# Nicolo2277/Vivim

Measured on AMD Instinct MI355X. Metric: frames/sec fwd+bwd, 256x256 clip=5 3-class, higher is better.
Workload: dtype bf16

## Files before the change

### vivim_amd/_lib.py

```python
import collections
import ctypes
import os
import re
import subprocess

import torch

_HERE = os.path.dirname(os.path.abspath(__file__))
CSRC = os.path.join(_HERE, "csrc")
SO_PATH = os.environ.get("VIVIM_LIB") or os.path.join(CSRC, "libvivim_hip.so")
HEADER = os.path.join(os.path.dirname(_HERE), "include", "vivim_hip.h")
EXT_HEADER = os.path.join(os.path.dirname(_HERE), "include", "vivim_hip_ext.h")

i32, i64, vp = ctypes.c_int32, ctypes.c_int64, ctypes.c_void_p

STRUCT_NAMES = {
    "vivim_ssm_fwd_params": "SsmFwdParams", "vivim_ssm_bwd_params": "SsmBwdParams",
    "vivim_conv_fwd_params": "ConvFwdParams", "vivim_conv_bwd_params": "ConvBwdParams",
    "vivim_dwconv_params": "DwConvParams", "vivim_dwconv_wgrad_params": "DwConvWgradParams",
    "vivim_dir_params": "DirParams", "vivim_conv_update_params": "ConvUpdateParams",
    "vivim_state_update_params": "StateUpdateParams", "vivim_layernorm_params": "LayerNormParams",
    "vivim_wgrad_nt_params": "WgradNtParams", "vivim_add_layernorm_params": "AddLayerNormParams",
    "vivim_seg_loss_params": "SegLossParams", "vivim_seg_metrics_params": "SegMetricsParams",
    "vivim_upsample_params": "UpsampleParams",
# ... 143 lines not shown
    if _lib is None:
        if not os.path.exists(SO_PATH):
            raise ImportError(
                f"{SO_PATH} is missing: run `python -c 'import __graft_entry__ as g; g.build()'` "
                "(or `make -C vivim_amd/csrc`). vivim_amd has no fallback path.")
        L = ctypes.CDLL(SO_PATH)
        for name, e in ALL_ENTRY_POINTS.items():
            fn = getattr(L, name)
            fn.argtypes = ([ctypes.POINTER(e.struct)] if e.struct else []) + list(e.extra) + ([vp] if e.stream else [])
            fn.restype = e.restype
        if L.vivim_abi_version() != ABI_VERSION:
            raise ImportError("libvivim_hip.so ABI version mismatch")
        for which, st in enumerate(STRUCTS):
            if L.vivim_sizeof(which) != ctypes.sizeof(st):
                raise ImportError(f"struct layout mismatch for {st.__name__}: "
                                  f"C {L.vivim_sizeof(which)} vs ctypes {ctypes.sizeof(st)}")
        _lib = L
    return _lib


_ISIZE = {F32: 4, F16: 2, BF16: 2}


def algorithmic_bytes(name, P):
    name = name.removesuffix("_det")
    f = P.f if isinstance(P, (SsmBwdParams, ConvBwdParams)) else P
    if name.startswith("vivim_opt"):
        if name.endswith("finalise"):
            return 8 * P.total_blocks + 4 * OPT_STATE_WORDS
        n = sum(P.numel[i] for i in range(P.count) if P.grads[i])
        if name.endswith("_mw"):
            return 2 * n + 8 * P.n_blocks if name.endswith("stats_mw") else 28 * n
        return 4 * n + 8 * P.n_blocks if name.endswith("stats") else 28 * n
    if name.startswith("vivim_add_layernorm"):
        n = P.batch * P.seqlen * P.channels
        if not P.weight:
            return n * ((2 if name.endswith("fwd") else 1) * _ISIZE[P.itype] + _ISIZE[P.btype])
        if name.endswith("fwd"):
            return n * (2 * _ISIZE[P.itype] + _ISIZE[P.btype] + _ISIZE[P.otype]) + 8 * P.batch * P.seqlen + 8 * P.channels
        res = (_ISIZE[P.itype] if P.dres else 0) + (_ISIZE[P.otype] if P.dy else 0) + (_ISIZE[P.btype] if P.dbranch else 0)
        return n * (2 * _ISIZE[P.itype] + res) + 8 * P.batch * P.seqlen + 12 * P.channels
    if name.startswith("vivim_token_add_norm"):
        n, b, r = P.rows * P.channels, _ISIZE[P.btype], _ISIZE[P.rtype]
        stats = 8 * P.rows if P.mean and P.weight else 0
        small = (4 * (P.rows // P.rows_per_sample) if P.scale else 0) + (4 * P.channels if P.weight else 0)
        if name.endswith("fwd"):
            small += 4 * P.channels if P.weight and P.bias else 0
            return n * (b + (r if P.res else 0) + (r if P.res_out else 0) + (b if P.weight else 0)) + stats + small
        norm = bool(P.weight and P.dy)
        small += (4 * P.channels if norm and P.dweight else 0) + (4 * P.channels if norm and P.dbias else 0)
        return (n * ((r + b if norm else 0) + (r if P.dres else 0) + (r if P.dres_in else 0) + (b if P.dbranch else 0))
                + (stats if norm else 0) + small)
    if name.startswith("vivim_token_layernorm"):
        n = P.rows * P.channels
        stats = 8 * P.rows if P.mean else 0
        if name.endswith("fwd"):
            return n * (_ISIZE[P.itype] + _ISIZE[P.otype]) + stats
        return n * (2 * _ISIZE[P.itype] + _ISIZE[P.otype]) + stats + 12 * P.channels
    if name.startswith("vivim_decode_head"):
        px = sum(P.map_h[s] * P.map_w[s] for s in range(P.n_maps))
        return (P.batch * (px * P.hidden + P.classes * P.out_h * P.out_w) * _ISIZE[P.itype]
                + 4 * (P.hidden + P.classes * P.hidden + P.classes))
    if name.startswith("vivim_head_concat"):
        px = P.out_h * P.out_w
        maps = sum(P.map_c[s] * (P.map_h[s] * P.map_w[s] + px) for s in range(P.n_maps)) * _ISIZE[P.itype]
        return P.batch * (maps + sum(P.map_c[s] * px for s in range(P.n_maps) if P.keep[s]))
    if name.startswith("vivim_upsample"):
        return P.batch * P.channels * (P.in_h * P.in_w + P.out_h * P.out_w) * _ISIZE[P.itype]
    if name.startswith("vivim_seg_metrics"):
        n = P.batch * P.pixels
        return n * (P.classes * _ISIZE[P.itype] + (8 if P.ttype == 0 else 1) + (1 if P.pred else 0)) + 12 * P.batch * P.classes
    if name.startswith("vivim_structure_loss"):
        n = P.batch * P.height * P.width
        return (n * ((2 if name.endswith("bwd") else 1) * P.classes * _ISIZE[P.itype] + (8 if P.ttype == 0 else 1))
                + 12 * P.batch * P.classes)
    if name.startswith("vivim_seg_loss"):
        n = P.batch * P.pixels
        return (n * ((2 if name.endswith("bwd") else 1) * P.classes * _ISIZE[P.itype] + (8 if P.ttype == 0 else 1))
                + 8 * P.batch * P.classes)
    if name.startswith("vivim_binary_metrics"):
        n = P.batch * P.height * P.width
        return (3 * n * (_ISIZE[P.ptype] + _ISIZE.get(P.gtype, 1)) + P.batch * (72 + (4096 if P.hist else 0))
                + (160 if P.state else 0))
    if name.startswith("vivim_selective_scan"):
        s = _ISIZE[f.itype]
        act = f.batch * f.dim * f.seqlen * s
        bc = (f.batch * f.n_groups * f.dstate * f.seqlen) if f.is_variable_B else f.dim * f.dstate
        has_z = bool(f.z)
        if name.endswith("fwd_lean"):
            return (4 if has_z else 3) * act + 2 * bc * (s if f.is_variable_B else 4) + 4 * (f.dim * f.dstate + 2 * f.dim)
        if name.endswith("fwd"):
            n_act = 3 + (2 if has_z else 0)
            return n_act * act + 2 * bc * (s if f.is_variable_B else 4) + 4 * (f.dim * f.dstate + 2 * f.dim)
        n_act = 5 + (3 if has_z else 0) + (1 if (has_z and f.out_z) else 0)
        return (n_act * act + 2 * bc * (s if f.is_variable_B else 4) + 2 * bc * 4
                + 4 * (2 * f.dim * f.dstate + 4 * f.dim))
    if name.endswith("_update"):
        return 0
    if name.startswith("vivim_dir"):
        return 4 * P.batch * P.channels * P.seqlen * _ISIZE[P.itype]
    if name.startswith("vivim_dwconv"):
        act = P.batch * P.depth * P.height * P.width * P.channels * _ISIZE[P.itype]
        return 2 * act + 4 * P.channels * (P.kd * 9 + 1)
    if name.startswith("vivim_layernorm"):
        n = P.batch * P.seqlen * P.channels
        if name.endswith("fwd"):
            return n * (_ISIZE[P.itype] + _ISIZE[P.otype]) + 8 * P.batch * P.seqlen + 8 * P.channels
        return n * (2 * _ISIZE[P.itype] + _ISIZE[P.otype]) + 8 * P.batch * P.seqlen + 12 * P.channels
    if name.startswith("vivim_wgrad"):
        return P.groups * ((P.m + P.n) * P.k * _ISIZE[P.itype] + 4 * P.m * P.n)
    s = _ISIZE[f.itype]
    act = f.batch * f.dim * f.seqlen * s
    if name.endswith("fwd"):
        return 2 * act + 4 * f.dim * (f.width + 1)
    return 3 * act + 8 * f.dim * (f.width + 1)


_profile = None
_event_pool = []
_PROFILED = ("vivim_selective_scan_fwd", "vivim_selective_scan_bwd", "vivim_causal_conv1d_fwd",
             "vivim_causal_conv1d_bwd")


def profile_begin(all_kernels=False):
    global _profile
    _profile = ([], bool(all_kernels))


def profile_end():
    global _profile
    rec = _profile[0] if _profile else []
    _profile = None
    out = []
    for name, nbytes, e0, e1 in rec:
        e1.synchronize()
        out.append((name, nbytes, e0.elapsed_time(e1) * 1e-3))
        _event_pool.extend((e0, e1))
    return out


def _event():
    if _event_pool:
        return _event_pool.pop()
    return torch.cuda.Event(enable_timing=True)


GUARD = os.environ.get("VIVIM_GUARD", "0") not in ("0", "")
_GUARD_BYTES = 1 << 16
_guards = []


def _guarded_storage(nbytes, device):
    buf = torch.full((nbytes + 2 * _GUARD_BYTES,), 0xA5, dtype=torch.uint8, device=device)
    _guards.append(buf)
    return buf[_GUARD_BYTES:_GUARD_BYTES + nbytes]


def empty(shape, dtype, device):
    if not GUARD:
        return torch.empty(shape, dtype=dtype, device=device)
    n = 1
    for d in shape:
        n *= d
    return _guarded_storage(n * torch.empty((), dtype=dtype).element_size(), device).view(dtype).view(shape)


# ... 71 lines not shown
```

### vivim_amd/csrc/capi.hip

```cpp
#include <hip/hip_runtime.h>
#include <float.h>
#include <stdarg.h>
#include <stddef.h>
#include <stdio.h>
#include <string.h>
#include <type_traits>
#include "ops.cuh"

using vivim::Launch;
using vivim::conv_channel_last;
using vivim::elem_bytes;
using vivim::vec_elems;

static thread_local char g_err[512] = "";

static int fail(int code, const char* fmt, ...) {
    va_list ap;
    va_start(ap, fmt);
    vsnprintf(g_err, sizeof(g_err), fmt, ap);
    va_end(ap);
    return code;
}

#define VCHECK(cond)                                                                   \
// ... 917 lines not shown
                    (long long)out_image);
    for (int s = 0; s < p->n_maps; ++s) {
        const int64_t image = (int64_t)p->map_c[s] * p->map_h[s] * p->map_w[s], mask = (int64_t)p->map_c[s] * p->out_h * p->out_w;
        const int64_t have = bwd ? p->dmap_batch_stride[s] : p->map_batch_stride[s];
        if (have < image)
            return fail(VIVIM_ERR_INVALID, "%s: %s[%d] = %lld: an image of map %d has %lld elements", fn,
                        bwd ? "dmap_batch_stride" : "map_batch_stride", s, (long long)have, s, (long long)image);
        if (p->keep[s] != nullptr && p->keep_batch_stride[s] < mask)
            return fail(VIVIM_ERR_INVALID, "%s: keep_batch_stride[%d] = %lld: a mask of map %d has %lld bytes", fn, s,
                        (long long)p->keep_batch_stride[s], s, (long long)mask);
    }
    bool fits = out_image <= INT32_MAX - 256 && (int64_t)p->batch * p->out_h <= INT32_MAX;
    for (int s = 0; s < p->n_maps; ++s)
        fits = fits && (2 * (int64_t)p->map_h[s] + 3) * p->out_h <= INT32_MAX && (2 * (int64_t)p->map_w[s] + 3) * p->out_w <= INT32_MAX;
    if (!fits || vivim::head_concat_blocks(*p, bwd) > INT32_MAX)
        return fail(VIVIM_ERR_INVALID, "%s: batch = %d, out (%d, %d), out_pixel_stride = %lld: the index range overflows int32", fn, p->batch,
                    p->out_h, p->out_w, (long long)p->out_pixel_stride);
    return VIVIM_OK;
}

int vivim_head_concat_fwd(const vivim_head_concat_params* p, void* stream) {
    const char* fn = "head_concat_fwd";
    if (int rc = check_head_concat(p, fn, false)) return rc;
    if (!vivim::head_concat_dispatch(*p, false, as_stream(stream)))
        return fail(VIVIM_ERR_UNSUPPORTED, "%s not implemented for type %d", fn, p->itype);
    return after_launch(fn);
}

int vivim_head_concat_bwd(const vivim_head_concat_params* p, void* stream) {
    const char* fn = "head_concat_bwd";
    if (int rc = check_head_concat(p, fn, true)) return rc;
    if (!vivim::head_concat_dispatch(*p, true, as_stream(stream)))
        return fail(VIVIM_ERR_UNSUPPORTED, "%s not implemented for type %d", fn, p->itype);
    return after_launch(fn);
}


static int check_binary_metrics(const vivim_binary_metrics_params* p, const char* fn) {
    if (p == nullptr) return fail(VIVIM_ERR_INVALID, "%s: params is NULL", fn);
    if (int rc = check_struct_bytes(fn, "vivim_binary_metrics_params", p->struct_bytes, sizeof(*p))) return rc;
    if (!dtype_ok(p->ptype)) return fail(VIVIM_ERR_INVALID, "%s: ptype = %d: pred is fp32 / fp16 / bf16 (0 / 1 / 2)", fn, p->ptype);
    if (!dtype_ok(p->gtype) && p->gtype != 3)
        return fail(VIVIM_ERR_INVALID, "%s: gtype = %d: gt is fp32 / fp16 / bf16 (0 / 1 / 2) or uint8 / bool (3)", fn, p->gtype);
    if (p->batch <= 0 || p->height <= 0 || p->width <= 0)
        return fail(VIVIM_ERR_INVALID, "%s: batch = %d, height = %d, width = %d: every size must be positive", fn, p->batch, p->height, p->width);
    const int64_t pixels = (int64_t)p->height * p->width;
    if (pixels < 2) return fail(VIVIM_ERR_INVALID, "%s: height * width = %lld: the metrics need at least 2 pixels", fn, (long long)pixels);
    if (pixels > INT32_MAX - 4096 || (int64_t)p->batch * 32 > INT32_MAX)
        return fail(VIVIM_ERR_INVALID, "%s: batch = %d, height * width = %lld: the index range overflows int32", fn, p->batch, (long long)pixels);
    if (p->pred_batch_stride < pixels || p->gt_batch_stride < pixels)
        return fail(VIVIM_ERR_INVALID, "%s: pred_batch_stride = %lld, gt_batch_stride = %lld: an image has %lld elements", fn,
                    (long long)p->pred_batch_stride, (long long)p->gt_batch_stride, (long long)pixels);
    return VIVIM_OK;
}

size_t vivim_binary_metrics_workspace_bytes(const vivim_binary_metrics_params* p) {
    if (check_binary_metrics(p, "binary_metrics_workspace_bytes") != VIVIM_OK) return 0;
    return vivim::binary_metrics_workspace_bytes(*p);
}

int vivim_binary_metrics(const vivim_binary_metrics_params* p, void* stream) {
    const char* fn = "binary_metrics";
    if (int rc = check_binary_metrics(p, fn)) return rc;
    if (p->pred == nullptr || !aligned(p->pred, elem_bytes(p->ptype)))
        return fail(VIVIM_ERR_INVALID, "%s: pred at %p: need a %d-byte aligned pointer", fn, p->pred, elem_bytes(p->ptype));
    const int gbytes = p->gtype == 3 ? 1 : elem_bytes(p->gtype);
    if (p->gt == nullptr || !aligned(p->gt, gbytes))
        return fail(VIVIM_ERR_INVALID, "%s: gt at %p: need a %d-byte aligned pointer", fn, p->gt, gbytes);
    if (p->thresholds == nullptr || !aligned(p->thresholds, 4))
        return fail(VIVIM_ERR_INVALID, "%s: thresholds at %p: need 256 fp32 thresholds at a 4-byte aligned pointer", fn, p->thresholds);
    if (p->values == nullptr || !aligned(p->values, 8))
        return fail(VIVIM_ERR_INVALID, "%s: values at %p: need an 8-byte aligned pointer to (batch, 9) fp64", fn, p->values);
    if (p->hist != nullptr && !aligned(p->hist, 4))
        return fail(VIVIM_ERR_INVALID, "%s: hist at %p: need NULL or a 4-byte aligned pointer", fn, p->hist);
    if (p->state != nullptr && !aligned(p->state, 8))
        return fail(VIVIM_ERR_INVALID, "%s: state at %p: need NULL or an 8-byte aligned pointer to 10 fp64", fn, p->state);
    const size_t need = vivim::binary_metrics_workspace_bytes(*p);
    if (int rc = check_workspace(fn, "vivim_binary_metrics_workspace_bytes", p->workspace, p->workspace_bytes, 8, need)) return rc;
    if (!vivim::binary_metrics_dispatch(*p, as_stream(stream)))
        return fail(VIVIM_ERR_UNSUPPORTED, "%s not implemented for type %d", fn, p->ptype);
    return after_launch(fn);
}

}
```

### vivim_amd/csrc/ops.cuh

```cuda
#pragma once
#include "det.cuh"
#include "../../include/vivim_hip_ext.h"
#include "../../include/vivim_hip_ext_head.h"
#include "../../include/vivim_hip_ext_binary_metrics.h"

namespace vivim {

inline bool conv_channel_last(const vivim_conv_fwd_params& f) { return f.x_c_stride == 1 && f.x_l_stride > 1; }
bool conv_fwd_dispatch(const vivim_conv_fwd_params&, hipStream_t);
bool conv_bwd_dispatch(const vivim_conv_bwd_params&, hipStream_t);
size_t conv_bwd_det_workspace_bytes(const vivim_conv_fwd_params&);
Launch conv_bwd_det_dispatch(const vivim_conv_bwd_params&, void* ws, size_t bytes, hipStream_t);
bool conv_cl_fwd_dispatch(const vivim_conv_fwd_params&, hipStream_t);
bool conv_cl_bwd_dispatch(const vivim_conv_bwd_params&, hipStream_t);
size_t conv_cl_bwd_det_slots(const vivim_conv_fwd_params&);
bool conv_cl_bwd_det_launch(const vivim_conv_bwd_params&, hipStream_t);

bool ssm_fwd_dispatch(const vivim_ssm_fwd_params&, hipStream_t);
bool ssm_fwd_lean_dispatch(const vivim_ssm_fwd_params&, void* last_state, hipStream_t);
bool ssm_bwd_dispatch(const vivim_ssm_bwd_params&, hipStream_t);
Launch ssm_bwd_det_dispatch(const vivim_ssm_bwd_params&, void* det_ws, size_t det_ws_bytes, hipStream_t);
int scan_chunk_len(int itype);
int scan_ckpt_len(const vivim_ssm_fwd_params&);
size_t scan_fwd_workspace_bytes(const vivim_ssm_fwd_params&);
size_t scan_bwd_workspace_bytes(const vivim_ssm_fwd_params&);
size_t scan_bwd_det_workspace_bytes(const vivim_ssm_fwd_params&);
size_t scan_bwd_det_call_workspace_bytes(const vivim_ssm_bwd_params&);

void conv_update_launch(const vivim_conv_update_params&, hipStream_t);
void state_update_launch(const vivim_state_update_params&, hipStream_t);

bool dwconv_fwd_dispatch(const vivim_dwconv_params&, hipStream_t);
bool dwconv_wgrad_dispatch(const vivim_dwconv_wgrad_params&, hipStream_t);
size_t dwconv_wgrad_det_workspace_bytes(const vivim_dwconv_wgrad_params&);
Launch dwconv_wgrad_det_dispatch(const vivim_dwconv_wgrad_params&, void* ws, size_t bytes, hipStream_t);

template <bool GATHER> bool dir_dispatch(const vivim_dir_params&, hipStream_t);

bool layernorm_dispatch(const vivim_layernorm_params&, bool bwd, hipStream_t);
size_t layernorm_bwd_workspace_bytes(const vivim_layernorm_params&);
bool add_layernorm_dispatch(const vivim_add_layernorm_params&, bool bwd, hipStream_t);
size_t add_layernorm_bwd_workspace_bytes(const vivim_add_layernorm_params&);

bool token_layernorm_dispatch(const vivim_token_layernorm_params&, bool bwd, hipStream_t);
bool token_layernorm_pair_ok(int itype, int otype);
size_t token_layernorm_bwd_workspace_bytes(const vivim_token_layernorm_params&);
bool token_add_norm_dispatch(const vivim_token_add_norm_params&, bool bwd, hipStream_t);
bool token_add_norm_pair_ok(int btype, int rtype);
size_t token_add_norm_bwd_workspace_bytes(const vivim_token_add_norm_params&);

bool wgrad_nt_dispatch(const vivim_wgrad_nt_params&, hipStream_t);

bool seg_loss_dispatch(const vivim_seg_loss_params&, bool bwd, hipStream_t);
size_t seg_loss_workspace_bytes(const vivim_seg_loss_params&);
bool seg_metrics_dispatch(const vivim_seg_metrics_params&, hipStream_t);
size_t seg_metrics_workspace_bytes(const vivim_seg_metrics_params&);
bool structure_loss_dispatch(const vivim_structure_loss_params&, bool bwd, hipStream_t);
size_t structure_loss_workspace_bytes(const vivim_structure_loss_params&);
int64_t structure_loss_tiles(const vivim_structure_loss_params&);

bool upsample_dispatch(const vivim_upsample_params&, bool bwd, hipStream_t);
int64_t upsample_blocks(const vivim_upsample_params&, bool bwd);
bool decode_head_dispatch(const vivim_decode_head_params&, hipStream_t);
int64_t decode_head_blocks(const vivim_decode_head_params&);
int decode_head_max_hidden();

bool head_concat_dispatch(const vivim_head_concat_params&, bool bwd, hipStream_t);
int64_t head_concat_blocks(const vivim_head_concat_params&, bool bwd);

bool binary_metrics_dispatch(const vivim_binary_metrics_params&, hipStream_t);
size_t binary_metrics_workspace_bytes(const vivim_binary_metrics_params&);

void opt_grad_stats_launch(const vivim_opt_step_params&, hipStream_t);
void opt_finalise_launch(const vivim_opt_step_params&, hipStream_t);
void opt_adamw_launch(const vivim_opt_step_params&, hipStream_t);
void opt_grad_stats_mw_launch(const vivim_opt_step_params&, int dtype, hipStream_t);
void opt_adamw_mw_launch(const vivim_opt_step_params&, const void* masters, int dtype, hipStream_t);

}
```

### vivim_amd/vivim.py

```python
import math

import os

import torch
import torch.nn as nn
import torch.nn.functional as F

from . import decode_head as _dh
from . import dwconv as _dw
from . import head_concat as _hc
from . import layernorm as _ln
from . import upsample as _up
from .mamba_simple import Mamba


class DropPath(nn.Module):

    def __init__(self, drop_prob=0.0):
        super().__init__()
        self.drop_prob = drop_prob

    def forward(self, x):
        if self.drop_prob == 0.0 or not self.training:
            return x
        keep = 1.0 - self.drop_prob
        mask = x.new_empty((x.shape[0],) + (1,) * (x.dim() - 1)).bernoulli_(keep).div_(keep)
        return x * mask

    def sample_scale(self, x):
        if self.drop_prob == 0.0 or not self.training:
            return None
        keep = 1.0 - self.drop_prob
        return torch.empty(x.shape[0], dtype=torch.float32, device=x.device).bernoulli_(keep).div_(keep)


def _init_weights(m):
    if isinstance(m, nn.Linear):
        nn.init.trunc_normal_(m.weight, std=0.02)
        if m.bias is not None:
            nn.init.constant_(m.bias, 0)
    elif isinstance(m, nn.LayerNorm):
        nn.init.constant_(m.bias, 0)
        nn.init.constant_(m.weight, 1.0)
    elif isinstance(m, nn.Conv2d):
        fan_out = m.kernel_size[0] * m.kernel_size[1] * m.out_channels // m.groups
        m.weight.data.normal_(0, math.sqrt(2.0 / fan_out))
        if m.bias is not None:
            m.bias.data.zero_()


class LayerNorm(nn.Module):

    def __init__(self, normalized_shape, eps=1e-6, data_format="channels_last"):
        super().__init__()
        if data_format not in ("channels_last", "channels_first"):
            raise NotImplementedError
        self.weight = nn.Parameter(torch.ones(normalized_shape))
        self.bias = nn.Parameter(torch.zeros(normalized_shape))
        self.eps = eps
        self.data_format = data_format
        self.normalized_shape = (normalized_shape,)

    def forward(self, x):
        if self.data_format == "channels_last":
            return F.layer_norm(x, self.normalized_shape, self.weight, self.bias, self.eps)
        mean = x.mean(1, keepdim=True)
        var = (x - mean).pow(2).mean(1, keepdim=True)
        x = (x - mean) / torch.sqrt(var + self.eps)
        return self.weight[:, None, None] * x + self.bias[:, None, None]


class DWConv(nn.Module):

    def __init__(self, dim=768):
        super().__init__()
        self.dwconv = nn.Conv3d(dim, dim, 3, 1, 1, bias=True, groups=dim)

    def forward(self, x, nf, H, W):
        B, _, C = x.shape
        if _dw.supported(x, self.dwconv.weight):
            return _dw.depthwise_conv_tokens(x, self.dwconv.weight, self.dwconv.bias, nf, H, W)
        x = self.dwconv(x.transpose(1, 2).view(B, C, nf, H, W))
        return x.flatten(2).transpose(1, 2)


class Mlp(nn.Module):
    def __init__(self, in_features, hidden_features=None, out_features=None, act_layer=nn.GELU, drop=0.0):
        super().__init__()
        out_features = out_features or in_features
        hidden_features = hidden_features or in_features
        self.fc1 = nn.Linear(in_features, hidden_features)
        self.dwconv = DWConv(hidden_features)
        self.act = act_layer()
        self.fc2 = nn.Linear(hidden_features, out_features)
        self.drop = nn.Dropout(drop)
        self.apply(_init_weights)

    def forward(self, x, nf, H, W):
        x = self.fc1(x)
        conv = self.dwconv.dwconv
        if isinstance(self.act, nn.GELU) and self.act.approximate == "none" and _dw.supported(x, conv.weight) \
                and not os.environ.get("VIVIM_NO_DWCONV_GELU"):
            x = self.drop(_dw.depthwise_conv_gelu_tokens(x, conv.weight, conv.bias, nf, H, W))
        else:
            x = self.drop(self.act(self.dwconv(x, nf, H, W)))
        return self.drop(self.fc2(x))


class MambaLayer(nn.Module):

    def __init__(self, dim, d_state=16, d_conv=4, expand=2, mlp_ratio=4, drop=0.0, drop_path=0.0,
                 act_layer=nn.GELU, fused_add_norm=False):
        super().__init__()
        self.dim = dim
        self.fused_add_norm = fused_add_norm
        self.norm1 = nn.LayerNorm(dim)
        self.mamba = Mamba(d_model=dim, d_state=d_state, d_conv=d_conv, expand=expand, bimamba_type="v3")
        self.drop_path = DropPath(drop_path) if drop_path > 0.0 else nn.Identity()
        self.norm2 = nn.LayerNorm(dim)
        self.mlp = Mlp(in_features=dim, hidden_features=int(dim * mlp_ratio), act_layer=act_layer, drop=drop)
        self.apply(_init_weights)

    @staticmethod
    def _norm(norm, x_flat):
        if (_ln.supported(x_flat, norm.weight) and _ln.worthwhile(x_flat)
                and not os.environ.get("VIVIM_NO_FUSED_LAYERNORM")):
            return _ln.layer_norm_cm(x_flat, norm.weight, norm.bias, norm.eps)
        return norm(x_flat)

    def forward(self, x):
        B, C, nf, H, W = x.shape
        assert C == self.dim
        x_flat = x.reshape(B, C, nf * H * W).transpose(-1, -2)
        branch = self.mamba(self._norm(self.norm1, x_flat), nframes=nf)
        if self.fused_add_norm and self._add_norm_applies(x_flat, branch, self.norm2.weight):
            x_flat, h = _ln.add_layer_norm_cm(x_flat, branch, self.norm2.weight, self.norm2.bias, self.norm2.eps,
                                              self._drop_scale(x_flat))
            branch = self.mlp(h, nf, H, W)
            if self._add_norm_applies(x_flat, branch, None):
                x_flat = _ln.add_cm(x_flat, branch, self._drop_scale(x_flat))
            else:
                x_flat = x_flat + self.drop_path(branch)
            return x_flat.transpose(-1, -2).reshape(B, C, nf, H, W)
        x_flat = x_flat + self.drop_path(branch)
        x_flat = x_flat + self.drop_path(self.mlp(self._norm(self.norm2, x_flat), nf, H, W))
        return x_flat.transpose(-1, -2).reshape(B, C, nf, H, W)

    @staticmethod
    def _add_norm_applies(x_flat, branch, weight):
        return (_ln.add_norm_supported(x_flat, branch, weight) and _ln.worthwhile(x_flat)
                and not os.environ.get("VIVIM_NO_FUSED_LAYERNORM"))

    def _drop_scale(self, x_flat):
        return self.drop_path.sample_scale(x_flat) if isinstance(self.drop_path, DropPath) else None


def _encoder_parts(backbone):
    seg = backbone.segformer
    if hasattr(seg, "encoder"):
        enc = seg.encoder
        return list(enc.patch_embeddings), list(enc.block), list(enc.layer_norm)
    return ([s.patch_embeddings for s in seg.stages], [s.blocks for s in seg.stages],
            [s.layer_norm for s in seg.stages])


class _TokenDWConv2d(nn.Module):

    def __init__(self, hf_module):
        super().__init__()
        self.dwconv = hf_module.dwconv

    def forward(self, hidden_states, height, width):
        if _dw.supported(hidden_states, self.dwconv.weight):
            return _dw.depthwise_conv_tokens(hidden_states, self.dwconv.weight, self.dwconv.bias, 1, height, width)
        b, _, c = hidden_states.shape
        y = self.dwconv(hidden_states.transpose(1, 2).view(b, c, height, width))
        return y.flatten(2).transpose(1, 2)


def _swap_backbone_dwconv(module):
    n = 0
    for m in module.modules():
        inner = getattr(m, "dwconv", None)
        conv = getattr(inner, "dwconv", None)
        if isinstance(conv, nn.Conv2d) and conv.groups == conv.in_channels and conv.kernel_size == (3, 3) \
                and conv.stride == (1, 1) and conv.padding == (1, 1) and not isinstance(inner, _TokenDWConv2d):
            m.dwconv = _TokenDWConv2d(inner)
            n += 1
    return n


def _swap_backbone_droppath(module):
    n = 0
    for m in module.modules():
        dp = getattr(m, "drop_path", None)
        if isinstance(dp, nn.Module) and type(dp).__name__ == "SegformerDropPath":
            m.drop_path = DropPath(float(dp.drop_prob))
            n += 1
    return n


class _BackboneLayerNorm(nn.LayerNorm):
    low_precision_out = False

    @classmethod
    def adopt(cls, norm, low_precision_out):
        new = cls(norm.normalized_shape, eps=norm.eps, elementwise_affine=False)
        new.elementwise_affine = norm.elementwise_affine
        new.weight, new.bias = norm.weight, norm.bias
        new.low_precision_out = low_precision_out
        new.train(norm.training)
        return new

    def forward(self, x):
        w, b = self.weight, self.bias
        if os.environ.get("VIVIM_NO_FUSED_LAYERNORM") or w is None or len(self.normalized_shape) != 1:
            return super().forward(x)
        low = torch.get_autocast_dtype("cuda") if self.low_precision_out and x.is_cuda and torch.is_autocast_enabled("cuda") else None
        if _ln.supported(x, w) and _ln.worthwhile(x):
            return _ln.layer_norm_cm(x, w, b, self.eps, out_dtype=low if low == x.dtype else None)
        rows = _ln.tm_rows(x, w, b)
        if rows is not None and _ln.tm_worthwhile(x):
            return _ln.layer_norm_tm(x, w, b, self.eps, out_dtype=low if low is not None and _ln.tm_pair_ok(x.dtype, low) else None,
                                     rows=rows)
        return super().forward(x)


def _swap_backbone_layernorm(encoder):
    n = 0
    for root, low in ((encoder.patch_embeddings, False), (encoder.block, True)):
        for m in root.modules():
            for name, child in list(m.named_children()):
                if isinstance(child, nn.LayerNorm) and not isinstance(child, _BackboneLayerNorm):
                    setattr(m, name, _BackboneLayerNorm.adopt(child, low))
                    n += 1
    return n


class _Encoder(nn.Module):

    def __init__(self, backbone):
        super().__init__()
        pe, blocks, norms = _encoder_parts(backbone)
        self.patch_embeddings = nn.ModuleList(pe)
        self.block = nn.ModuleList(blocks)
        self.layer_norm = nn.ModuleList(norms)


def _run_block(blk, hs, height, width):
    out = blk(hs, height, width)
    return out[0] if isinstance(out, (tuple, list)) else out


def _block_norms(blk):
    for first, second in (("layernorm_before", "layernorm_after"), ("layer_norm_1", "layer_norm_2")):
        n1, n2 = getattr(blk, first, None), getattr(blk, second, None)
        if isinstance(n1, nn.LayerNorm) and isinstance(n2, nn.LayerNorm):
            ok = all(isinstance(getattr(blk, name, None), nn.Module) for name in ("attention", "mlp", "drop_path"))
            return (n1, n2) if ok else None
    return None


def _add_rows(res, branch, drop_path, norm=None):
    if not isinstance(drop_path, (DropPath, nn.Identity)):
        return None
    w = b = None
    if norm is not None:
        w, b = norm.weight, norm.bias
        if w is None or len(norm.normalized_shape) != 1:
            return None
        want = torch.get_autocast_dtype("cuda") if res.is_cuda and torch.is_autocast_enabled("cuda") else res.dtype
        if branch.dtype != want:
            return None
    rows = _ln.tm_add_rows(res, branch, w, b)
    return rows if rows is not None and _ln.tm_add_worthwhile(res) else None


def _add_norm_site(res, branch, drop_path, norm):
    rows = _add_rows(res, branch, drop_path, norm)
    if rows is None:
        h = drop_path(branch) + res
        return h, norm(h)
    scale = drop_path.sample_scale(branch) if isinstance(drop_path, DropPath) else None
    return _ln.add_layer_norm_tm(res, branch, norm.weight, norm.bias, norm.eps, scale=scale, rows=rows)


def _add_site(res, branch, drop_path):
    rows = _add_rows(res, branch, drop_path)
    if rows is None:
        return drop_path(branch) + res
    scale = drop_path.sample_scale(branch) if isinstance(drop_path, DropPath) else None
    return _ln.add_tm(res, branch, scale=scale, rows=rows)


def _run_stage(blocks, hs, height, width):
    pending = None
    for blk in blocks:
        norms = _block_norms(blk)
        if norms is None:
            if pending is not None:
                hs, pending = _add_site(*pending), None
            hs = _run_block(blk, hs, height, width)
            continue
        if pending is None:
            y = norms[0](hs)
        else:
            hs, y = _add_norm_site(*pending, norms[0])
        branch = blk.attention(y, height, width)
        if isinstance(branch, (tuple, list)):
            branch = branch[0]
        dropout = getattr(blk, "hidden_dropout", None)
        if dropout is not None:
            branch = dropout(branch)
        hs, y = _add_norm_site(hs, branch, blk.drop_path, norms[1])
        pending = (hs, blk.mlp(y, height, width), blk.drop_path)
    return hs if pending is None else _add_site(*pending)


class mamba_block(nn.Module):

    def __init__(self, backbone, in_chans=1, depths=[2, 2, 2, 2], dims=[64, 128, 320, 512],
                 drop_path_rate=0.0, layer_scale_init_value=1e-6, out_indices=[0, 1, 2, 3], mamba_kwargs=None,
                 fast_backbone_dwconv=False, fast_backbone_layernorm=False, fused_backbone_add_norm=False):
        super().__init__()
        self.downsample_layers = _Encoder(backbone)
        self.fused_backbone_add_norm = fused_backbone_add_norm
        if fast_backbone_dwconv:
            _swap_backbone_dwconv(self.downsample_layers)
        if fast_backbone_dwconv or fused_backbone_add_norm:
            _swap_backbone_droppath(self.downsample_layers)
        if fast_backbone_layernorm:
            _swap_backbone_layernorm(self.downsample_layers)
        dp_rates = [x.item() for x in torch.linspace(0, drop_path_rate, sum(depths))]
        mk = mamba_kwargs or {}
        self.stages = nn.ModuleList()
        for i in range(len(dims)):
            self.stages.append(nn.Sequential(*[nn.Sequential(MambaLayer(dim=dims[i], drop_path=dp_rates[i], **mk))
                                               for _ in range(depths[i])]))
        self.out_indices = out_indices

    def forward_features(self, x):
        bz, nf = x.shape[:2]
        hs = x.reshape(bz * nf, *x.shape[-3:])
        outs = []
        enc = self.downsample_layers
        for embed, blocks, _norm, mam_stage in zip(enc.patch_embeddings, enc.block, enc.layer_norm, self.stages):
            hs, height, width = embed(hs)
            if self.fused_backbone_add_norm and not os.environ.get("VIVIM_NO_FUSED_LAYERNORM"):
                hs = _run_stage(blocks, hs, height, width)
            else:
                for blk in blocks:
                    hs = _run_block(blk, hs, height, width)
            hs = hs.reshape(bz * nf, height, width, -1).permute(0, 3, 1, 2).contiguous()
            hs = hs.reshape(bz, nf, *hs.shape[-3:]).transpose(1, 2)
            hs = mam_stage(hs)
            hs = hs.transpose(1, 2).reshape(bz * nf, hs.shape[1], height, width)
            outs.append(hs)
        return tuple(outs)

    def forward(self, x):
        return self.forward_features(x)


def segformer_b3_config(num_labels=150):
    from transformers import SegformerConfig
    return SegformerConfig(num_channels=3, num_encoder_blocks=4, depths=[3, 4, 18, 3], sr_ratios=[8, 4, 2, 1],
                           hidden_sizes=[64, 128, 320, 512], patch_sizes=[7, 3, 3, 3], strides=[4, 2, 2, 2],
                           num_attention_heads=[1, 2, 5, 8], mlp_ratios=[4, 4, 4, 4], decoder_hidden_size=768,
                           num_labels=num_labels)


def segformer_b3_random(num_labels=150):
    from transformers import SegformerForSemanticSegmentation
    return SegformerForSemanticSegmentation(segformer_b3_config(num_labels))


class Vivim(nn.Module):

    def __init__(self, in_chans=3, out_chans=3, depths=[2, 2, 2, 2], feat_size=[64, 128, 320, 512],
                 drop_path_rate=0.2, layer_scale_init_value=1e-6, hidden_size: int = 768, norm_name="instance",
                 conv_block: bool = True, res_block: bool = True, spatial_dims=2, with_edge=False,
                 dropout_rate=0.3, backbone=None, mamba_kwargs=None, fast_backbone_dwconv=False,
                 fused_upsample=False, fused_decode_head=False, fast_backbone_layernorm=False,
                 fused_backbone_add_norm=False, fused_head_concat=False) -> None:
        super().__init__()
        self.fused_upsample = fused_upsample
        self.fused_head_concat = fused_head_concat
        self.fused_decode_head = fused_decode_head
        self.hidden_size = hidden_size
        self.in_chans, self.out_chans = in_chans, out_chans
        self.depths, self.feat_size = depths, feat_size
        self.drop_path_rate = drop_path_rate
        self.layer_scale_init_value = layer_scale_init_value
        self.dropout_rate = dropout_rate
        self.spatial_dims = spatial_dims
        if backbone is None:
            from transformers import SegformerForSemanticSegmentation
            backbone = SegformerForSemanticSegmentation.from_pretrained("nvidia/segformer-b3-finetuned-ade-512-512")
        self.encoder = mamba_block(backbone, in_chans, depths=depths, dims=feat_size,
                                   drop_path_rate=drop_path_rate, mamba_kwargs=mamba_kwargs,
                                   fast_backbone_dwconv=fast_backbone_dwconv,
                                   fast_backbone_layernorm=fast_backbone_layernorm,
                                   fused_backbone_add_norm=fused_backbone_add_norm)
        self.decoder = backbone.decode_head
        self.feature_dropout = nn.Dropout2d(dropout_rate)
        self.out = nn.Conv2d(768, out_chans, kernel_size=1)
        self.with_edge = with_edge
        if with_edge:
            self.edgeocr_cls_head = nn.Conv2d(64, 1, kernel_size=1, stride=1, padding=0, bias=True)

    def _upsample(self, x, size):
        if self.fused_upsample:
            return _up.bilinear_upsample(x, size)
# ... 46 lines not shown
```

Baseline: 216.3.

## Add split-K fp32 linear weight-gradient kernel and route MLP and backbone linears through it

Adds a HIP kernel that computes a linear layer's fp32 weight and bias gradients from 16-bit activations and output gradients. It splits the token dimension across workgroups, accumulates 64x64 tiles per wave in registers via LDS staging, and combines the partials with a separate reduce kernel. A custom autograd function keeps the forward in autocast dtype and uses this kernel in backward for large token counts. The aim is to replace the autocast matmul plus dtype cast plus bias-reduction path with one fused pass that writes fp32 gradients directly. The cost is a split workspace, an extra reduce launch, and a CUDA-core FMA loop that may lose to a tuned library GEMM.

```diff
diff --git a/include/vivim_hip_ext_linear_wgrad.h b/include/vivim_hip_ext_linear_wgrad.h
--- /dev/null
+++ b/include/vivim_hip_ext_linear_wgrad.h
@@ -0,0 +1,29 @@
+#ifndef VIVIM_HIP_EXT_LINEAR_WGRAD_H
+#define VIVIM_HIP_EXT_LINEAR_WGRAD_H
+
+#include "vivim_hip.h"
+
+#ifdef __cplusplus
+extern "C" {
+#endif
+
+typedef struct {
+    int32_t struct_bytes;
+    int32_t tokens, in_features, out_features;
+    int32_t itype;
+    int32_t splits;
+    int64_t x_row_stride, dy_row_stride;
+    const void *x, *dy;
+    void *dweight;
+    void *dbias;
+    void *workspace;
+    int64_t workspace_bytes;
+} vivim_linear_wgrad_params;
+
+size_t vivim_linear_wgrad_workspace_bytes(const vivim_linear_wgrad_params *p);
+int vivim_linear_wgrad(const vivim_linear_wgrad_params *p, void *stream);
+
+#ifdef __cplusplus
+}
+#endif
+#endif
diff --git a/vivim_amd/_lib.py b/vivim_amd/_lib.py
--- a/vivim_amd/_lib.py
+++ b/vivim_amd/_lib.py
@@ -249,6 +249,8 @@
         n = P.batch * P.height * P.width
         return (3 * n * (_ISIZE[P.ptype] + _ISIZE.get(P.gtype, 1)) + P.batch * (72 + (4096 if P.hist else 0))
                 + (160 if P.state else 0))
+    if name.startswith("vivim_linear_wgrad"):
+        return (P.in_features + P.out_features) * P.tokens * _ISIZE[P.itype] + 4 * P.out_features * (P.in_features + (1 if P.dbias else 0))
     if name.startswith("vivim_selective_scan"):
         s = _ISIZE[f.itype]
         act = f.batch * f.dim * f.seqlen * s
diff --git a/vivim_amd/csrc/capi.hip b/vivim_amd/csrc/capi.hip
--- a/vivim_amd/csrc/capi.hip
+++ b/vivim_amd/csrc/capi.hip
@@ -1023,4 +1023,46 @@
     return after_launch(fn);
 }
 
-}
+
+static int check_linear_wgrad(const vivim_linear_wgrad_params* p, const char* fn) {
+    if (p == nullptr) return fail(VIVIM_ERR_INVALID, "%s: params is NULL", fn);
+    if (int rc = check_struct_bytes(fn, "vivim_linear_wgrad_params", p->struct_bytes, sizeof(*p))) return rc;
+    if (p->itype != VIVIM_F16 && p->itype != VIVIM_BF16)
+        return fail(VIVIM_ERR_UNSUPPORTED, "%s: itype = %d: x and dy are fp16 or bf16 (1 / 2)", fn, p->itype);
+    if (p->tokens <= 0 || p->in_features <= 0 || p->out_features <= 0 || p->splits < 0)
+        return fail(VIVIM_ERR_INVALID, "%s: tokens = %d, in_features = %d, out_features = %d, splits = %d: sizes must be positive, splits >= 0",
+                    fn, p->tokens, p->in_features, p->out_features, p->splits);
+    if (p->in_features % 8 != 0 || p->out_features % 8 != 0)
+        return fail(VIVIM_ERR_INVALID, "%s: in_features = %d, out_features = %d: need multiples of 8 (16-byte vectors)", fn, p->in_features,
+                    p->out_features);
+    if (p->x_row_stride < p->in_features || p->dy_row_stride < p->out_features || p->x_row_stride % 8 != 0 || p->dy_row_stride % 8 != 0)
+        return fail(VIVIM_ERR_INVALID, "%s: x_row_stride = %lld, dy_row_stride = %lld: need multiples of 8 that hold a row", fn,
+                    (long long)p->x_row_stride, (long long)p->dy_row_stride);
+    if (p->tokens > (1 << 30) || p->in_features > (1 << 15) || p->out_features > (1 << 15) || vivim::linear_wgrad_tiles(*p) > 65535)
+        return fail(VIVIM_ERR_INVALID, "%s: tokens = %d, in_features = %d, out_features = %d: the index range overflows", fn, p->tokens,
+                    p->in_features, p->out_features);
+    return VIVIM_OK;
+}
+
+size_t vivim_linear_wgrad_workspace_bytes(const vivim_linear_wgrad_params* p) {
+    if (check_linear_wgrad(p, "linear_wgrad_workspace_bytes") != VIVIM_OK) return 0;
+    return vivim::linear_wgrad_workspace_bytes(*p);
+}
+
+int vivim_linear_wgrad(const vivim_linear_wgrad_params* p, void* stream) {
+    const char* fn = "linear_wgrad";
+    if (int rc = check_linear_wgrad(p, fn)) return rc;
+    if (p->x == nullptr || p->dy == nullptr || !aligned16(p->x) || !aligned16(p->dy))
+        return fail(VIVIM_ERR_INVALID, "%s: x at %p, dy at %p: need 16-byte aligned pointers", fn, p->x, p->dy);
+    if (p->dweight == nullptr || !aligned16(p->dweight))
+        return fail(VIVIM_ERR_INVALID, "%s: dweight at %p: need a 16-byte aligned pointer to (out_features, in_features) fp32", fn, p->dweight);
+    if (p->dbias != nullptr && !aligned16(p->dbias))
+        return fail(VIVIM_ERR_INVALID, "%s: dbias at %p: need NULL or a 16-byte aligned pointer", fn, p->dbias);
+    const size_t need = vivim::linear_wgrad_workspace_bytes(*p);
+    if (int rc = check_workspace(fn, "vivim_linear_wgrad_workspace_bytes", p->workspace, p->workspace_bytes, 16, need)) return rc;
+    if (!vivim::linear_wgrad_dispatch(*p, as_stream(stream)))
+        return fail(VIVIM_ERR_UNSUPPORTED, "%s not implemented for type %d", fn, p->itype);
+    return after_launch(fn);
+}
+
+}
diff --git a/vivim_amd/csrc/linear_wgrad.hip b/vivim_amd/csrc/linear_wgrad.hip
--- /dev/null
+++ b/vivim_amd/csrc/linear_wgrad.hip
@@ -0,0 +1,200 @@
+#include "ops.cuh"
+
+namespace vivim {
+
+constexpr int kLwWaves = 8;
+constexpr int kLwThreads = kLwWaves * kWave;
+constexpr int kLwTile = 64;
+constexpr int kLwStep = 8;
+constexpr int kLwRound = kLwWaves * kLwStep;
+constexpr int kLwTargetWgs = 256;
+constexpr int kLwRedGroups = 16;
+constexpr int kLwRedVecs = 16;
+
+typedef float lw_f2 __attribute__((ext_vector_type(2)));
+typedef float lw_f4 __attribute__((ext_vector_type(4)));
+
+struct LwPlan {
+    int out_tiles, in_tiles, splits, rounds_per_split;
+    int64_t slot_elems;
+};
+
+static LwPlan lw_plan(const vivim_linear_wgrad_params& p) {
+    LwPlan q;
+    q.out_tiles = (p.out_features + kLwTile - 1) / kLwTile;
+    q.in_tiles = (p.in_features + kLwTile - 1) / kLwTile;
+    const int rounds = (p.tokens + kLwRound - 1) / kLwRound;
+    int want = p.splits > 0 ? p.splits : std::max(1, kLwTargetWgs / (q.out_tiles * q.in_tiles));
+    want = std::min(want, rounds);
+    q.rounds_per_split = (rounds + want - 1) / want;
+    q.splits = (rounds + q.rounds_per_split - 1) / q.rounds_per_split;
+    q.slot_elems = (int64_t)p.out_features * p.in_features + p.out_features;
+    return q;
+}
+
+template <typename T> __device__ __forceinline__ void lw_widen(const u32x4 v, float (&f)[8]) {
+    union { u32x4 raw; T e[8]; } u;
+    u.raw = v;
+#pragma unroll
+    for (int k = 0; k < 8; ++k) f[k] = to_f32<T>(u.e[k]);
+}
+
+template <typename T>
+__global__ void __launch_bounds__(kLwThreads) linear_wgrad_partial_kernel(const vivim_linear_wgrad_params p, const int rounds_per_split,
+                                                                          const int in_tiles, const int64_t slot_elems) {
+    __shared__ __attribute__((aligned(16))) float tile[kLwWaves][kLwTile * kLwTile];
+    __shared__ __attribute__((aligned(16))) float dbl[kLwWaves][kLwStep][kLwTile];
+    const int tid = threadIdx.x, w = tid >> 6, lane = tid & 63;
+    const int i = lane >> 3, j = lane & 7;
+    const int ot = blockIdx.y / in_tiles, it = blockIdx.y - ot * in_tiles;
+    const int out0 = ot * kLwTile, in0 = it * kLwTile;
+    const bool with_db = p.dbias != nullptr && it == 0;
+    const int k0 = blockIdx.x * rounds_per_split * kLwRound;
+    const int k1 = min(p.tokens, k0 + rounds_per_split * kLwRound);
+
+    const T* __restrict__ xb = static_cast<const T*>(p.x);
+    const T* __restrict__ dyb = static_cast<const T*>(p.dy);
+    const bool dy_ch = out0 + 8 * j < p.out_features, x_ch = in0 + 8 * j < p.in_features;
+    const u32x4 zero = {0u, 0u, 0u, 0u};
+    auto load = [&](int round, u32x4& rdy, u32x4& rx) {
+        const int t = k0 + round * kLwRound + w * kLwStep + i;
+        const bool vdy = t < k1 && dy_ch, vx = t < k1 && x_ch;
+        const u32x4 a = *reinterpret_cast<const u32x4*>(vdy ? dyb + (int64_t)t * p.dy_row_stride + out0 + 8 * j : dyb);
+        const u32x4 b = *reinterpret_cast<const u32x4*>(vx ? xb + (int64_t)t * p.x_row_stride + in0 + 8 * j : xb);
+        rdy = vdy ? a : zero;
+        rx = vx ? b : zero;
+    };
+
+    lw_f2 acc[8][4];
+#pragma unroll
+    for (int a = 0; a < 8; ++a)
+#pragma unroll
+        for (int b = 0; b < 4; ++b) acc[a][b] = lw_f2{0.f, 0.f};
+    float dbacc[8];
+#pragma unroll
+    for (int c = 0; c < 8; ++c) dbacc[c] = 0.f;
+
+    u32x4* stage = reinterpret_cast<u32x4*>(&tile[w][0]);
+    u32x4 rdy[2], rx[2];
+    load(0, rdy[0], rx[0]);
+    load(1, rdy[1], rx[1]);
+    for (int r = 0; r < rounds_per_split; r += 2) {
+#pragma unroll
+        for (int h = 0; h < 2; ++h) {
+            u32x4* buf = stage + h * (kLwStep * 16);
+            buf[i * 16 + j] = rdy[h];
+            buf[i * 16 + 8 + j] = rx[h];
+            if (with_db) {
+                float f[8];
+                lw_widen<T>(rdy[h], f);
+#pragma unroll
+                for (int c = 0; c < 8; ++c) dbacc[c] += f[c];
+            }
+            load(r + h + 2, rdy[h], rx[h]);
+            wave_lds_fence();
+#pragma unroll
+            for (int tt = 0; tt < kLwStep; ++tt) {
+                float d[8], v[8];
+                lw_widen<T>(buf[tt * 16 + i], d);
+                lw_widen<T>(buf[tt * 16 + 8 + j], v);
+#pragma unroll
+                for (int a = 0; a < 8; ++a) {
+                    const lw_f2 da = {d[a], d[a]};
+#pragma unroll
+                    for (int b = 0; b < 4; ++b) acc[a][b] = __builtin_elementwise_fma(da, lw_f2{v[2 * b], v[2 * b + 1]}, acc[a][b]);
+                }
+            }
+            wave_lds_fence();
+        }
+    }
+
+    float* mine = tile[w];
+#pragma unroll
+    for (int a = 0; a < 8; ++a) {
+        lw_f4* dst = reinterpret_cast<lw_f4*>(mine + (8 * i + a) * kLwTile + 8 * j);
+        dst[0] = lw_f4{acc[a][0].x, acc[a][0].y, acc[a][1].x, acc[a][1].y};
+        dst[1] = lw_f4{acc[a][2].x, acc[a][2].y, acc[a][3].x, acc[a][3].y};
+    }
+    if (with_db) {
+#pragma unroll
+        for (int c = 0; c < 8; ++c) dbl[w][i][8 * j + c] = dbacc[c];
+    }
+    __syncthreads();
+    float* __restrict__ slot = static_cast<float*>(p.workspace) + (int64_t)blockIdx.x * slot_elems;
+    const int e = tid * 8, orow = out0 + (e >> 6), icol = in0 + (e & 63);
+    lw_f4 s0 = *reinterpret_cast<const lw_f4*>(&tile[0][e]), s1 = *reinterpret_cast<const lw_f4*>(&tile[0][e + 4]);
+#pragma unroll
+    for (int ww = 1; ww < kLwWaves; ++ww) {
+        s0 += *reinterpret_cast<const lw_f4*>(&tile[ww][e]);
+        s1 += *reinterpret_cast<const lw_f4*>(&tile[ww][e + 4]);
+    }
+    if (orow < p.out_features && icol < p.in_features) {
+        lw_f4* dst = reinterpret_cast<lw_f4*>(slot + (int64_t)orow * p.in_features + icol);
+        dst[0] = s0;
+        dst[1] = s1;
+    }
+    if (with_db && tid < kLwTile && out0 + tid < p.out_features) {
+        float s = 0.f;
+#pragma unroll
+        for (int ww = 0; ww < kLwWaves; ++ww)
+#pragma unroll
+            for (int row = 0; row < kLwStep; ++row) s += dbl[ww][row][tid];
+        slot[(int64_t)p.out_features * p.in_features + out0 + tid] = s;
+    }
+}
+
+__global__ void __launch_bounds__(kLwRedGroups * kLwRedVecs) linear_wgrad_reduce_kernel(const float* __restrict__ ws, const int splits,
+                                                                                       const int64_t slot_elems, const int64_t n_dw,
+                                                                                       const int64_t n_total, float* __restrict__ dw,
+                                                                                       float* __restrict__ db) {
+    __shared__ lw_f4 part[kLwRedGroups][kLwRedVecs];
+    const int ev = threadIdx.x % kLwRedVecs, sg = threadIdx.x / kLwRedVecs;
+    const int64_t e = ((int64_t)blockIdx.x * kLwRedVecs + ev) * 4;
+    const int per = (splits + kLwRedGroups - 1) / kLwRedGroups;
+    const int s_lo = sg * per, s_hi = min(splits, s_lo + per);
+    lw_f4 s = {0.f, 0.f, 0.f, 0.f};
+    if (e < n_total) {
+#pragma unroll 4
+        for (int k = s_lo; k < s_hi; ++k) s += *reinterpret_cast<const lw_f4*>(ws + (int64_t)k * slot_elems + e);
+    }
+    part[sg][ev] = s;
+    __syncthreads();
+    if (sg == 0 && e < n_total) {
+        lw_f4 t = part[0][ev];
+#pragma unroll
+        for (int g = 1; g < kLwRedGroups; ++g) t += part[g][ev];
+        *reinterpret_cast<lw_f4*>(e < n_dw ? dw + e : db + (e - n_dw)) = t;
+    }
+}
+
+size_t linear_wgrad_workspace_bytes(const vivim_linear_wgrad_params& p) {
+    const LwPlan q = lw_plan(p);
+    return (size_t)q.splits * (size_t)q.slot_elems * sizeof(float);
+}
+
+int64_t linear_wgrad_tiles(const vivim_linear_wgrad_params& p) {
+    const LwPlan q = lw_plan(p);
+    return (int64_t)q.out_tiles * q.in_tiles;
+}
+
+template <typename T> static void lw_launch(const vivim_linear_wgrad_params& p, const LwPlan& q, hipStream_t stream) {
+    hipLaunchKernelGGL((linear_wgrad_partial_kernel<T>), dim3(q.splits, q.out_tiles * q.in_tiles), dim3(kLwThreads), 0, stream, p,
+                       q.rounds_per_split, q.in_tiles, q.slot_elems);
+}
+
+bool linear_wgrad_dispatch(const vivim_linear_wgrad_params& p, hipStream_t stream) {
+    const LwPlan q = lw_plan(p);
+    switch (p.itype) {
+        case VIVIM_BF16: lw_launch<bf16_t>(p, q, stream); break;
+        case VIVIM_F16: lw_launch<f16_t>(p, q, stream); break;
+        default: return false;
+    }
+    const int64_t n_dw = (int64_t)p.out_features * p.in_features, n_total = n_dw + (p.dbias ? p.out_features : 0);
+    const int64_t blocks = (n_total + 4 * kLwRedVecs - 1) / (4 * kLwRedVecs);
+    hipLaunchKernelGGL(linear_wgrad_reduce_kernel, dim3((unsigned)blocks), dim3(kLwRedGroups * kLwRedVecs), 0, stream,
+                       static_cast<const float*>(p.workspace), q.splits, q.slot_elems, n_dw, n_total, static_cast<float*>(p.dweight),
+                       static_cast<float*>(p.dbias));
+    return true;
+}
+
+}
diff --git a/vivim_amd/csrc/ops.cuh b/vivim_amd/csrc/ops.cuh
--- a/vivim_amd/csrc/ops.cuh
+++ b/vivim_amd/csrc/ops.cuh
@@ -3,6 +3,7 @@
 #include "../../include/vivim_hip_ext.h"
 #include "../../include/vivim_hip_ext_head.h"
 #include "../../include/vivim_hip_ext_binary_metrics.h"
+#include "../../include/vivim_hip_ext_linear_wgrad.h"
 
 namespace vivim {
 
@@ -51,6 +52,10 @@
 
 bool wgrad_nt_dispatch(const vivim_wgrad_nt_params&, hipStream_t);
 
+bool linear_wgrad_dispatch(const vivim_linear_wgrad_params&, hipStream_t);
+size_t linear_wgrad_workspace_bytes(const vivim_linear_wgrad_params&);
+int64_t linear_wgrad_tiles(const vivim_linear_wgrad_params&);
+
 bool seg_loss_dispatch(const vivim_seg_loss_params&, bool bwd, hipStream_t);
 size_t seg_loss_workspace_bytes(const vivim_seg_loss_params&);
 bool seg_metrics_dispatch(const vivim_seg_metrics_params&, hipStream_t);
diff --git a/vivim_amd/linear_wgrad.py b/vivim_amd/linear_wgrad.py
--- /dev/null
+++ b/vivim_amd/linear_wgrad.py
@@ -0,0 +1,135 @@
+import ctypes
+import os
+import types
+
+import torch
+import torch.nn.functional as F
+
+from . import _lib
+from . import wgrad as _wgrad
+
+HEADER = os.path.join(os.path.dirname(_lib.HEADER), "vivim_hip_ext_linear_wgrad.h")
+STRUCT_NAMES = {"vivim_linear_wgrad_params": "LinearWgradParams"}
+_, _classes, ENTRY_POINTS = _lib.parse_header(_lib._read_header(HEADER), STRUCT_NAMES)
+LinearWgradParams = _classes["LinearWgradParams"]
+_ITYPE = {torch.float16: _lib.F16, torch.bfloat16: _lib.BF16}
+MIN_TOKENS = max(15360, _wgrad.MIN_TOKENS)
+_bound = False
+_ws_bytes = {}
+
+
+def _bind():
+    global _bound
+    if not _bound:
+        L = _lib.lib()
+        for name, e in ENTRY_POINTS.items():
+            fn = getattr(L, name)
+            fn.argtypes = ([ctypes.POINTER(e.struct)] if e.struct else []) + list(e.extra) + ([_lib.vp] if e.stream else [])
+            fn.restype = e.restype
+        _bound = True
+
+
+def _rows_ok(t):
+    return t.stride(1) == 1 and (t.shape[0] == 1 or t.stride(0) % 8 == 0) and t.data_ptr() % 16 == 0
+
+
+def shapes_ok(x, weight, bias, dtype=None):
+    if not (torch.is_tensor(x) and x.dim() >= 2 and (dtype or x.dtype) in _ITYPE and x.numel() > 0 and x.stride(-1) == 1):
+        return False
+    if not (weight.dim() == 2 and weight.dtype == torch.float32 and weight.is_contiguous() and weight.shape[1] == x.shape[-1]):
+        return False
+    if bias is not None and not (bias.dtype == torch.float32 and bias.is_contiguous() and bias.shape == (weight.shape[0],)):
+        return False
+    out, inn = weight.shape
+    return out % 8 == 0 and inn % 8 == 0 and out <= 1 << 15 and inn <= 1 << 15 and x.numel() // inn <= 1 << 30
+
+
+def supported(x, weight, bias):
+    if os.environ.get("VIVIM_NO_LINEAR_WGRAD") or not (torch.is_tensor(x) and x.is_cuda and torch.is_grad_enabled()):
+        return False
+    if not (weight.requires_grad and weight.device == x.device and (bias is None or bias.device == x.device)):
+        return False
+    if not torch.is_autocast_enabled("cuda"):
+        return False
+    dtype = torch.get_autocast_dtype("cuda")
+    if x.dtype not in (dtype, torch.float32) or not shapes_ok(x, weight, bias, dtype):
+        return False
+    return x.dtype != dtype or x.data_ptr() % 16 == 0
+
+
+def worthwhile(tokens):
+    return tokens >= MIN_TOKENS
+
+
+def linear_wgrad(x, dy, bias=True, splits=0):
+    _bind()
+    _lib.check(x.dim() == 2 and dy.dim() == 2 and x.shape[0] == dy.shape[0] and x.dtype == dy.dtype and x.dtype in _ITYPE
+               and x.is_cuda and dy.device == x.device, "linear_wgrad: x (K, in) and dy (K, out) of one 16-bit dtype on one GPU")
+    K, inn = x.shape
+    out = dy.shape[1]
+    dev = x.device
+    P = LinearWgradParams()
+    P.struct_bytes = ctypes.sizeof(P)
+    P.tokens, P.in_features, P.out_features, P.itype, P.splits = K, inn, out, _ITYPE[x.dtype], splits
+    P.x_row_stride, P.dy_row_stride = (x.stride(0) if K > 1 else inn), (dy.stride(0) if K > 1 else out)
+    P.x, P.dy = x.data_ptr(), dy.data_ptr()
+    key = (K, inn, out, splits)
+    ws_bytes = _ws_bytes.get(key)
+    if ws_bytes is None:
+        ws_bytes = _lib.lib().vivim_linear_wgrad_workspace_bytes(P)
+        _lib.check(ws_bytes > 0, "vivim_linear_wgrad_workspace_bytes refused the shapes: " + _lib.lib().vivim_last_error().decode())
+        _ws_bytes[key] = ws_bytes
+    ws = _lib.empty((ws_bytes,), torch.uint8, dev)
+    dw = _lib.empty((out, inn), torch.float32, dev)
+    db = _lib.empty((out,), torch.float32, dev) if bias else None
+    P.dweight, P.dbias, P.workspace, P.workspace_bytes = dw.data_ptr(), _lib.ptr(db), _lib.ptr(ws), ws_bytes
+    _lib.launch("vivim_linear_wgrad", P, dev)
+    return dw, db
+
+
+class _LinearFn(torch.autograd.Function):
+    @staticmethod
+    @torch.amp.custom_fwd(device_type="cuda")
+    def forward(ctx, x, weight, bias):
+        w16 = weight.to(x.dtype)
+        b16 = None if bias is None else bias.to(x.dtype)
+        ctx.save_for_backward(x, w16)
+        ctx.has_bias = bias is not None
+        return F.linear(x, w16, b16)
+
+    @staticmethod
+    @torch.amp.custom_bwd(device_type="cuda")
+    def backward(ctx, dy):
+        x, w16 = ctx.saved_tensors
+        out, inn = w16.shape
+        dy2, x2 = dy.reshape(-1, out), x.reshape(-1, inn)
+        if not _rows_ok(dy2):
+            dy2 = dy2.contiguous()
+        if not _rows_ok(x2):
+            x2 = x2.contiguous()
+        dx = (dy2 @ w16).view(x.shape) if ctx.needs_input_grad[0] else None
+        dw = db = None
+        if ctx.needs_input_grad[1] or (ctx.has_bias and ctx.needs_input_grad[2]):
+            dw, db = linear_wgrad(x2, dy2, bias=ctx.has_bias and ctx.needs_input_grad[2])
+        return dx, dw, db
+
+
+def linear(x, weight, bias=None):
+    if x.dim() >= 2 and worthwhile(x.numel() // max(x.shape[-1], 1)) and supported(x, weight, bias):
+        dtype = torch.get_autocast_dtype("cuda")
+        return _LinearFn.apply(x if x.dtype == dtype else x.to(dtype), weight, bias)
+    return F.linear(x, weight, bias)
+
+
+def _forward(self, x):
+    return linear(x, self.weight, self.bias)
+
+
+def adopt(lin):
+    if not adopted(lin):
+        lin.forward = types.MethodType(_forward, lin)
+    return lin
+
+
+def adopted(lin):
+    return getattr(lin.__dict__.get("forward"), "__func__", None) is _forward
diff --git a/vivim_amd/vivim.py b/vivim_amd/vivim.py
--- a/vivim_amd/vivim.py
+++ b/vivim_amd/vivim.py
@@ -10,6 +10,7 @@
 from . import dwconv as _dw
 from . import head_concat as _hc
 from . import layernorm as _ln
+from . import linear_wgrad as _lw
 from . import upsample as _up
 from .mamba_simple import Mamba
 
@@ -89,10 +90,10 @@
         super().__init__()
         out_features = out_features or in_features
         hidden_features = hidden_features or in_features
-        self.fc1 = nn.Linear(in_features, hidden_features)
+        self.fc1 = _lw.adopt(nn.Linear(in_features, hidden_features))
         self.dwconv = DWConv(hidden_features)
         self.act = act_layer()
-        self.fc2 = nn.Linear(hidden_features, out_features)
+        self.fc2 = _lw.adopt(nn.Linear(hidden_features, out_features))
         self.drop = nn.Dropout(drop)
         self.apply(_init_weights)
 
@@ -196,6 +197,15 @@
         dp = getattr(m, "drop_path", None)
         if isinstance(dp, nn.Module) and type(dp).__name__ == "SegformerDropPath":
             m.drop_path = DropPath(float(dp.drop_prob))
+            n += 1
+    return n
+
+
+def _swap_backbone_linear(encoder):
+    n = 0
+    for m in encoder.block.modules():
+        if type(m) is nn.Linear and not _lw.adopted(m):
+            _lw.adopt(m)
             n += 1
     return n
 
@@ -329,6 +339,8 @@
             _swap_backbone_dwconv(self.downsample_layers)
         if fast_backbone_dwconv or fused_backbone_add_norm:
             _swap_backbone_droppath(self.downsample_layers)
+        if fast_backbone_dwconv:
+            _swap_backbone_linear(self.downsample_layers)
         if fast_backbone_layernorm:
             _swap_backbone_layernorm(self.downsample_layers)
         dp_rates = [x.item() for x in torch.linspace(0, drop_path_rate, sum(depths))]
```

New measurement: 213.5. -1.3%, worse.
